# kit-cel/vae-equalizer

Measured on AMD Instinct MI355X. Metric: equalized symbols/s/GPU, DP 64-QAM VAE-LE, higher is better.
Workload: dtype f32

## Files before the change

### vae_equalizer_amd/csrc/vaeq_dp_wave_kernel.h

```cpp
#pragma once
#include <hip/hip_runtime.h>
#include <stdint.h>
#include <type_traits>

#include "vaeq.h"
#include "vaeq_common.h"
#include "vaeq_launch.h"
#include "vaeq_wave.h"

#ifdef VAEQ_PHASE_STAMPS
#define VAEQ_STAMP(i) do { if (s == a.steps - 1) tst[i] = __builtin_readcyclecounter(); } while (0)
#define VAEQ_XSTAMP(i) do { if (s == a.steps - 1) tsx[i] = __builtin_readcyclecounter(); } while (0)
#else
#define VAEQ_STAMP(i) do { } while (0)
#define VAEQ_XSTAMP(i) do { } while (0)
#endif
#define VAEQ_NSTAMP 12
#ifndef VAEQ_PIPE
#define VAEQ_PIPE 1
#endif
#define VAEQ_BT_FRAMES 16
#ifndef VAEQ_WPS
#define VAEQ_WPS 2
#endif
// ... 6 lines not shown
    return __builtin_bit_cast(float, (unsigned)r[0]) + __builtin_bit_cast(float, (unsigned)r[1]);
}

struct WaveLayout {
    int Lph, Uph;
    int X, E, U, PSv, W, H, PSh, VS, MOM, RED, XG, total;
};

__host__ __device__ inline WaveLayout wave_layout(int B, int M, int NW = 1)
{
    WaveLayout l;
    const int len = 2 * B + M - 1;
    const int lph = wave_lph(len);
    l.Lph = lph;
    l.Uph = B / 2 + 1;
    int o = 0;
    auto take = [&](int bytes) { int r = o; o += (bytes + 15) & ~15; return r; };
    l.X = take(2 * 4 * lph * 8);
    l.E = take(2 * 4 * lph * 8);
    const int ubytes = 2 * 2 * l.Uph * 8, gbytes = 2 * B * 8;
    l.U = take(ubytes > gbytes ? ubytes : gbytes);
    l.PSv = take(2 * (B + 1) * 4);
    l.W = take(2 * M * 16);
    l.H = take(2 * 2 * (M + 1) * 8);
    l.PSh = take(2 * (M + 1) * 4);
    l.VS = take(2 * M * 4);
    l.MOM = take(16 * 64 * 4);
    l.RED = take(NW > 1 ? 64 * 4 : 0);
    l.XG = take((NW - 1) * 4 * 64 * 4);
    l.total = o;
    return l;
}

template <int M, bool INIT, bool PIPE = true, bool SPLIT = true>
__device__ __forceinline__ void pair_fir(cacc (&acc)[2][2], cacc (&accx)[2][2], const float2 *xp, int Lph, const float4 *wq)
{
    cacc (&acc2)[2][2] = SPLIT ? accx : acc;
    auto tapA = [&](int k) -> v2f { return lds2(reinterpret_cast<const float2 *>(wq + k)); };
    auto tapB = [&](int k) -> v2f { return lds2(reinterpret_cast<const float2 *>(wq + k) + 1); };
    constexpr int G = M / 4;
    auto load = [&](int g, v2f (&r)[14]) {
        const float2 *xg = xp + g;
        r[0] = lds2(xg); r[1] = lds2(xg + Lph); r[2] = lds2(xg + 2 * Lph); r[3] = lds2(xg + 3 * Lph); r[4] = lds2(xg + 1); r[5] = lds2(xg + Lph + 1);
#pragma unroll
        for (int t = 0; t < 4; t++) { r[6 + 2 * t] = tapA(4 * g + t); r[7 + 2 * t] = tapB(4 * g + t); }
    };
    auto fma = [&](int, const v2f (&r)[14], auto first) {
        constexpr bool F = decltype(first)::value;
        cmacf<F>(acc[0][0], r[6], r[0]); cmacf<F>(acc[0][1], r[7], r[0]); cmacf<F>(acc[1][0], r[6], r[2]); cmacf<F>(acc[1][1], r[7], r[2]);
        cmacf<F && SPLIT>(acc2[0][0], r[8], r[1]); cmacf<F && SPLIT>(acc2[0][1], r[9], r[1]);
        cmacf<F && SPLIT>(acc2[1][0], r[8], r[3]); cmacf<F && SPLIT>(acc2[1][1], r[9], r[3]);
        cmac(acc[0][0], r[10], r[2]); cmac(acc[0][1], r[11], r[2]); cmac(acc[1][0], r[10], r[4]); cmac(acc[1][1], r[11], r[4]);
        cmac(acc2[0][0], r[12], r[3]); cmac(acc2[0][1], r[13], r[3]); cmac(acc2[1][0], r[12], r[5]); cmac(acc2[1][1], r[13], r[5]);
    };
    pipe2<14, INIT, PIPE>(G, load, fma);
#pragma unroll
    for (int k = 4 * G; k < M; k++) {
        const v2f a = tapA(k), b = tapB(k);
        const v2f xa = lds2(xp + (k & 3) * Lph + (k >> 2)), xb = lds2(xp + ((k + 2) & 3) * Lph + ((k + 2) >> 2));
        if (k & 1) { cmac(acc2[0][0], a, xa); cmac(acc2[0][1], b, xa); cmac(acc2[1][0], a, xb); cmac(acc2[1][1], b, xb); }
        else { cmac(acc[0][0], a, xa); cmac(acc[0][1], b, xa); cmac(acc[1][0], a, xb); cmac(acc[1][1], b, xb); }
    }
}

template <int M, bool MERGE = true>
__device__ __forceinline__ void pair_du(cacc (&acc)[2][2][2], const float2 *ep, int Lph, const float2 *ht, int MP)
{
    constexpr int G = M / 4;
    auto load1 = [&](int chi, int g, v2f *x) {
        const float2 *xg = ep + chi * 4 * Lph + g;
        x[0] = lds2(xg); x[1] = lds2(xg + Lph); x[2] = lds2(xg + 2 * Lph); x[3] = lds2(xg + 3 * Lph); x[4] = lds2(xg + 1); x[5] = lds2(xg + Lph + 1);
#pragma unroll
        for (int t = 0; t < 4; t++) { x[6 + 2 * t] = lds2(ht + (chi * 2 + 0) * MP + 4 * g + t); x[7 + 2 * t] = lds2(ht + (chi * 2 + 1) * MP + 4 * g + t); }
    };
    auto fma1 = [&](int chi, const v2f *x, int t, auto first) {
        constexpr bool F = decltype(first)::value;
        cmacf<F>(acc[chi][0][0], x[6 + 2 * t], x[t]); cmacf<F>(acc[chi][0][1], x[7 + 2 * t], x[t]);
        cmacf<F>(acc[chi][1][0], x[6 + 2 * t], x[t + 2]); cmacf<F>(acc[chi][1][1], x[7 + 2 * t], x[t + 2]);
    };
    if constexpr (MERGE) {
        auto load = [&](int g, v2f (&r)[28]) { load1(0, g, r); load1(1, g, r + 14); };
        auto fma = [&](int, const v2f (&r)[28], auto first) {
            fma1(0, r, 0, first); fma1(1, r + 14, 0, first);
#pragma unroll
            for (int t = 1; t < 4; t++) { fma1(0, r, t, std::false_type{}); fma1(1, r + 14, t, std::false_type{}); }
        };
        pipe2<28, true, false>(G, load, fma);
    } else {
#pragma unroll
        for (int chi = 0; chi < 2; chi++) {
            auto load = [&](int g, v2f (&r)[14]) { load1(chi, g, r); };
            auto fma = [&](int, const v2f (&r)[14], auto first) {
                fma1(chi, r, 0, first);
#pragma unroll
                for (int t = 1; t < 4; t++) fma1(chi, r, t, std::false_type{});
            };
            pipe2<14, true, false>(G, load, fma);
        }
    }
#pragma unroll
    for (int k = 4 * G; k < M; k++)
#pragma unroll
        for (int chi = 0; chi < 2; chi++) {
            const float2 *xp = ep + chi * 4 * Lph;
            const v2f a = lds2(ht + (chi * 2 + 0) * MP + k), b = lds2(ht + (chi * 2 + 1) * MP + k);
            const v2f xa = lds2(xp + (k & 3) * Lph + (k >> 2)), xb = lds2(xp + ((k + 2) & 3) * Lph + ((k + 2) >> 2));
            cmac(acc[chi][0][0], a, xa); cmac(acc[chi][0][1], b, xa); cmac(acc[chi][1][0], a, xb); cmac(acc[chi][1][1], b, xb);
        }
}

constexpr bool uniform_parts(int B, int M, int NP)
{
    const int mh = M / 2, nm = 2 * B - 2 * mh;
// ... 146 lines not shown
    }
    constexpr bool LB = NST % 2 == 0;
    v2f t[6];
    if constexpr (N & 1) {
        constexpr int m = N - 1;
        t[0] = lds2(sA + SS * m); t[1] = lds2(sB + SS * m); t[2] = lds2(tA + m); t[3] = lds2(tA + TN + m); t[4] = lds2(tB + m); t[5] = lds2(tB + TN + m);
    }
    if constexpr (LB) { head(B, A, std::false_type{}); rest(B); }
    if constexpr (N & 1) {
        const v2f (&p)[12] = LB ? B : A;
        cmac(ca[1][0], p[10], t[0]); cmac(ca[1][1], p[11], t[0]); cmac(ca[0][0], t[2], t[0]); cmac(ca[0][1], t[3], t[0]);
        cmac(cb[0][0], t[4], t[1]); cmac(cb[0][1], t[5], t[1]); cmac(cb[1][0], t[2], t[1]); cmac(cb[1][1], t[3], t[1]);
    }
#pragma unroll
    for (int x = 0; x < 2; x++)
#pragma unroll
        for (int y = 0; y < 2; y++) { ca[x][y].a += cb[x][y].a; ca[x][y].b += cb[x][y].b; }
}

template <int M, int NLEV, int BT, bool PAIR, int OUT, int NW = 1, int BL = 0>
__global__ __launch_bounds__(64 * NW, VAEQ_WPS) void dp_wave_kernel(const vaeq_dp_args a)
{
    constexpr int mh = M / 2, Mh = 2 * mh, MP = M + 1;
    constexpr float LOG2E = 1.4426950408889634f, LN2 = 0.6931471805599453f;
    extern __shared__ float4 smem4[];
    char *sm = reinterpret_cast<char *>(smem4);
    const int gl = threadIdx.x, lane = NW > 1 ? (gl & 63) : gl, wv = NW > 1 ? (gl >> 6) : 0, run = blockIdx.x;
    constexpr int NT = 64 * NW, NP = 2 * NW;
    constexpr bool UNI = BT > 0 && uniform_parts(BT, M, NP);
    constexpr bool FIXL = BT > 0 || (BL > 0 && M != 13 && M != 17 && !(M == 31 && NW == 1));
    constexpr bool PIPE = VAEQ_PIPE && FIXL;
    constexpr bool WIDE = FIXL;
    constexpr bool B100 = BT == 100 && NW == 1;
    constexpr int QAUX = B100 ? 2 : 0;
    const int B = BT ? BT : a.B;
    const int BS = BT ? BT : BL ? BL : B;
    constexpr bool ODDB = BT == 0 && BL > 0;
    const int L = 2 * B, nm = L - Mh, P2 = ODDB ? (B + 1) / 2 : B / 2;
    const float rnm = 1.0f / (float)nm;
    const WaveLayout lay = wave_layout(BS, M, NW);
    const int Lph = lay.Lph, Uph = lay.Uph;
    float2 *Xs = reinterpret_cast<float2 *>(sm + lay.X), *Es = reinterpret_cast<float2 *>(sm + lay.E);
    float2 *Us = reinterpret_cast<float2 *>(sm + lay.U), *GY = Us;
    float4 *Wt = reinterpret_cast<float4 *>(sm + lay.W);
    float2 *Ht = reinterpret_cast<float2 *>(sm + lay.H);
    float *PSv = reinterpret_cast<float *>(sm + lay.PSv);
    float *PSh = reinterpret_cast<float *>(sm + lay.PSh);
    float *VS = reinterpret_cast<float *>(sm + lay.VS);
    float *RED = reinterpret_cast<float *>(sm + lay.RED), *XG = reinterpret_cast<float *>(sm + lay.XG);

    float amp[NLEV], b2[NLEV], nlogP[NLEV];
    const float nusc = a.nu_sc[run];
#pragma unroll
    for (int i = 0; i < NLEV; i++) {
        amp[i] = a.amp[i];
        b2[i] = nusc * amp[i] * amp[i] * LOG2E;
        nlogP[i] = -logf(a.P[(size_t)run * NLEV + i]);
    }
    const float var0 = a.var[run * 2 + 0], var1 = a.var[run * 2 + 1];
    const float lrW = a.lr_W[run], lrH = a.lr_h[run];

    for (int i = gl; i < (lay.W - lay.X) / 8; i += NT) Xs[i] = make_float2(0.f, 0.f);
    for (int i = gl; i < (lay.PSh - lay.H) / 8; i += NT) Ht[i] = make_float2(0.f, 0.f);
    __syncthreads();
    const int tk = lane & 31, half = lane >> 5;
    const bool worker = tk < M, owner = worker && wv == 0;
// ... 71 lines not shown
            b2t = BTW[1][f];
        }
        const bool qf = OUT != 2 && a.q_out, yf = a.y_out, ef = OUT != 1 && a.eq_out, df = OUT != 1 && a.dec_out;
        const uint32_t No4 = (uint32_t)No * 4u;
        const size_t fr = (size_t)run * a.n_frames + f;
        const __amdgpu_buffer_rsrc_t qr = make_rsrc(qf ? a.q_out + fr * (4 * NLEV) * No : nullptr, qf ? 4u * NLEV * No4 : 0u);
        const __amdgpu_buffer_rsrc_t yr = make_rsrc(yf ? a.y_out + fr * 4 * No : nullptr, yf ? 4u * No4 : 0u);
        const __amdgpu_buffer_rsrc_t er = make_rsrc(ef ? a.eq_out + fr * 2 * No : nullptr, ef ? 2u * No4 : 0u);
        const __amdgpu_buffer_rsrc_t dr = make_rsrc(df ? a.dec_out + fr * 4 * No : nullptr, df ? (uint32_t)(4 * No) : 0u);
        const __amdgpu_buffer_rsrc_t lr_ = make_rsrc(a.loss ? a.loss + fr * a.steps : nullptr, a.loss ? (uint32_t)a.steps * 4u : 0u);
        const __amdgpu_buffer_rsrc_t vr_ = make_rsrc(a.var_est ? a.var_est + fr * 2 * a.steps : nullptr, a.var_est ? (uint32_t)a.steps * 8u : 0u);
#pragma unroll 1
        for (int s = 0; s < a.steps; s++) {
            VAEQ_STAMP(0);
            if (ldl) {
#pragma unroll
                for (int p = 0; p < 2; p++) {
                    const float4 I4 = pf[p * 2 + 0], Q4 = pf[p * 2 + 1];
                    const float xi[4] = {I4.x, I4.y, I4.z, I4.w}, xq[4] = {Q4.x, Q4.y, Q4.z, Q4.w};
#pragma unroll
                    for (int i = 0; i < 4; i++) {
                        const int c = mh + i;
                        const bool in = !ODDB || 4 * gl + i < L;
                        Xs[(p * 4 + (c & 3)) * Lph + gl + (c >> 2)] = in ? make_float2(xi[i], xq[i]) : make_float2(0.f, 0.f);
                    }
                }
            }
            sync_lds<NW>();

            VAEQ_STAMP(1);
            float2 y[2][2];
            {
                cacc ya[2][2], yb[2][2];
                pair_fir<M, true, PIPE, WIDE>(ya, yb, Xa, Lph, Wt);
                pair_fir<M, false, PIPE, WIDE>(ya, yb, Xa + 4 * Lph, Lph, Wt + M);
#pragma unroll
                for (int sy = 0; sy < 2; sy++)
#pragma unroll
                    for (int o = 0; o < 2; o++) {
                        if constexpr (WIDE) {
                            ya[sy][o].a += yb[sy][o].a;
                            ya[sy][o].b += yb[sy][o].b;
                        }
                        y[sy][o] = cfin(ya[sy][o]);
                    }
            }
            asm volatile("" : "+v"(y[0][0].x), "+v"(y[0][0].y), "+v"(y[0][1].x), "+v"(y[0][1].y), "+v"(y[1][0].x), "+v"(y[1][0].y),
                         "+v"(y[1][1].x), "+v"(y[1][1].y));
            VAEQ_STAMP(2);
            const bool kept0 = act && (n0 >= k0) && (n0 < k0 + klen), kept1 = act && (n0 + 1 >= k0) && (n0 + 1 < k0 + klen);
            const uint32_t col = (uint32_t)(s * klen + (n0 - k0));
            const uint32_t vo0 = kept0 ? col * 4u : OOB, vo1 = kept1 ? col * 4u + 4u : OOB;
            if (yf) {
                uint32_t yrow = 0u;
                auto next_row = [&]() {
                    yrow += No4;
                    asm volatile("" : "+s"(yrow));
                };
#pragma unroll
                for (int o = 0; o < 2; o++) {
                    const uint32_t r0 = yrow;
                    next_row();
                    const uint32_t r1 = yrow;
                    next_row();
                    if (pairst) {
                        bst64(v2f{y[0][o].x, y[1][o].x}, yr, vo0, r0);
                        bst64(v2f{y[0][o].y, y[1][o].y}, yr, vo0, r1);
                    } else {
// ... 101 lines not shown
                    sync_lds<NW>();
#pragma unroll
                    for (int w = 0; w < NW - 1; w++)
                        if (w < wv) { inc[0] += RED[w]; inc[1] += RED[NW + w]; }
                }
#pragma unroll
                for (int o = 0; o < 2; o++) {
                    if (act) {
                        PSv[o * (BS + 1) + n0 + 1] = inc[o] - vv[o][1];
                        PSv[o * (BS + 1) + n0 + 2] = inc[o];
                    }
                    if (gl == 0) PSv[o * (BS + 1)] = 0.f;
                }
            }
            sync_lds<NW>();
            if (owner) {
                const int lo = (Mh - tk + 1) >> 1, hi_ = (nm - 1 + Mh - tk) >> 1;
                VS[half * M + tk] = PSv[half * (BS + 1) + hi_ + 1] - PSv[half * (BS + 1) + lo];
            }
            sync_lds<NW>();

            VAEQ_STAMP(5);
            float se0 = 0.f, se1 = 0.f;
            float hq0 = 0.f, hq1 = 0.f;
            if (worker) {
                const float2 h0 = Ht[(0 * 2 + half) * MP + tk], h1 = Ht[(1 * 2 + half) * MP + tk];
                hq0 = h0.x * h0.x + h0.y * h0.y;
                hq1 = h1.x * h1.x + h1.y * h1.y;
            }
            const float vsl = worker ? VS[half * M + tk] : 0.f;
            if constexpr (B100 && M == 25) {
                constexpr int T = 100 - mh, NB = (mh + 1) / 2;
                static_assert((mh & 1) == 0 && (Mh & 3) == 0 && D3Map::exact(100, M), "D3Map: mh even (a = mh stands alone, its odd tap is the pad)");
                int l3 = lane;
                asm volatile("" : "+v"(l3));
                const int m3 = D3Map::m(l3, T), modd = m3 & 1, m3h = (3 * m3) >> 1;
                cacc D3[3][2];
                const int xo = D3Map::chi(l3) * 4 * Lph + (Mh >> 2) + m3h;
                const int o0 = xo + (modd ? 2 * Lph : 0), o2 = xo + (modd ? 1 : 2 * Lph);
                const int off[6] = {o0, o0 + Lph, o2, o2 + Lph, o0 + 1, o0 + Lph + 1};
                v2f x6[6];
#pragma unroll
                for (int k = 0; k < 6; k++) x6[k] = lds2(Xs + off[k]);
                {
                    const float2 *uE = Us + modd * Uph + m3h, *uO = Us + (modd ^ 1) * Uph + m3h + modd;
                    const float2 *hc = Ht + D3Map::chi(l3) * 2 * MP;
                    v2f am[2][4];
#pragma unroll
                    for (int v = 0; v < 2; v++) {
                        am[v][0] = lds2(hc + v * MP + Mh);
                        am[v][1] = lds2(uE + v * 2 * Uph); am[v][2] = lds2(uO + v * 2 * Uph); am[v][3] = lds2(uE + v * 2 * Uph + 1);
                    }
#pragma unroll
                    for (int v = 0; v < 2; v++) {
                        const float2 *hv = hc + v * MP, *ue = uE + v * 2 * Uph, *uo = uO + v * 2 * Uph;
                        {
                            const v2f t = am[v][0], u0 = am[v][1], u1 = am[v][2], u2 = am[v][3];
                            if (v == 0) { cmul(D3[0][0], t, u0); cmul(D3[1][0], t, u1); cmul(D3[2][0], t, u2); }
                            else { cmac(D3[0][0], t, u0); cmac(D3[1][0], t, u1); cmac(D3[2][0], t, u2); }
                        }
                        auto load = [&](int b, v2f (&r)[8]) {
                            const int sl = (mh >> 1) - b;
                            r[0] = lds2(uo + sl - 1); r[1] = lds2(ue + sl); r[2] = lds2(uo + sl); r[3] = lds2(ue + sl + 1);
#pragma unroll
                            for (int t = 0; t < 4; t++) r[4 + t] = lds2(hv + 4 * b + t);
                        };
                        auto fma = [&](int, const v2f (&r)[8], auto first) {
                            constexpr bool F = decltype(first)::value;
                            v2f t0 = r[4], t1 = r[5], t2 = r[6], t3 = r[7];
                            asm volatile("" : "+v"(t0), "+v"(t1));
#pragma unroll
                            for (int i = 0; i < 3; i++) {
                                cmac(D3[i][0], t0, r[i + 1]);
                                cmacf<F>(D3[i][1], t1, r[i + 1]);
                                if constexpr (F) asm volatile("" : "+v"(D3[i][1].a), "+v"(D3[i][1].b));
                            }
                            asm volatile("" : "+v"(t2), "+v"(t3));
#pragma unroll
                            for (int i = 0; i < 3; i++) { cmac(D3[i][0], t2, r[i]); cmac(D3[i][1], t3, r[i]); }
                        };
                        if (v == 0) pipe2<8, true, PIPE>(NB, load, fma);
                        else pipe2<8, false, PIPE>(NB, load, fma);
                    }
                }
                VAEQ_STAMP(6);
                {
                    float2 e[6];
#pragma unroll
                    for (int k = 0; k < 6; k++) {
                        const float2 x = f2(x6[k]);
                        const float2 Dv = cfin(D3[k >> 1][k & 1]);
                        e[k] = make_float2(x.x - Dv.x, x.y - Dv.y);
                        if (6 * (D3Map::nm_lanes(T) - 1) + k >= 2 * T && 6 * m3 + k >= nm) e[k] = make_float2(0.f, 0.f);
                    }
                    if (D3Map::works(l3, T)) {
#pragma unroll
                        for (int k = 0; k < 6; k++) Es[off[k]] = e[k];
                    }
                }
                sync_lds<NW>();
                {
                    const float2 *Eq = Es + (gl < nq ? gl : 0);
                    v2f eq[2][4];
#pragma unroll
                    for (int chi = 0; chi < 2; chi++)
#pragma unroll
                        for (int i = 0; i < 4; i++) eq[chi][i] = lds2(Eq + (chi * 4 + ((Mh + i) & 3)) * Lph + ((Mh + i) >> 2));
#pragma unroll
                    for (int chi = 0; chi < 2; chi++)
#pragma unroll
                        for (int i = 0; i < 4; i++) {
                            const float2 e = f2(eq[chi][i]);
                            const float e2 = __builtin_fmaf(e.x, e.x, e.y * e.y);
                            if (chi) se1 += e2; else se0 += e2;
// ... 79 lines not shown
                }
            }
            {
                const float inc = half_incl_scan_dpp(gC0 * hq0 + gC1 * hq1);
                if (owner) PSh[half * MP + tk + 1] = inc;
                if (tk == 0) PSh[half * MP] = 0.f;
            }
            sync_lds<NW>();

            VAEQ_STAMP(7);
            step += 1;
            b1t *= 0.9;
            b2t *= 0.999;
            const float rbc1 = __builtin_amdgcn_rcpf((float)(1.0 - b1t));
            const float bc2s = __builtin_amdgcn_rcpf(__builtin_amdgcn_sqrtf((float)(1.0 - b2t)));
            const float ssW = lrW * rbc1, ssH = lrH * rbc1;
            float2 hnew[2];
            hnew[0] = hnew[1] = make_float2(0.f, 0.f);
            float ghr[2] = {0, 0}, ghi[2] = {0, 0};
            float2 hacc[2];
            {
                float2 ph_h[2] = {make_float2(0.f, 0.f), make_float2(0.f, 0.f)};
                float ph_vs[2] = {0.f, 0.f};
                if (NW == 1 && ownr) {
#pragma unroll
                    for (int v = 0; v < 2; v++) {
                        ph_h[v] = Ht[(oc * 2 + v) * MP + tj];
                        ph_vs[v] = VS[v * M + tj];
                    }
                }
                cacc ca[2][2];
                if constexpr (TP) {
                    static_assert(TapPairMap::exact(100, M) && UNI, "TapPairMap");
                    int lt = lane;
                    asm volatile("" : "+v"(lt));
                    constexpr int NH = TapPairMap::dh_pairs(100, M);
                    const int par = TapPairMap::par(lt, M), sl = TapPairMap::alo(lt, M) >> 1, ma = TapPairMap::part_h(lt, M) * NH;
                    const int ceA = par + Mh, ceB = par + Mh + 2;
                    const float2 *ec = Es + TapPairMap::c(lt, M) * 4 * Lph + ma;
                    const float2 *uA = Us + (mh >> 1) - sl + ma, *uB = uA + Uph;
                    const float2 *uC = TapPairMap::tap(lt, M, 1) < M ? uB - 1 : uA;
                    VAEQ_XSTAMP(0);
                    tap_pair_sum<NH, 1>(ca, ec + (ceA & 3) * Lph + (ceA >> 2), ec + (ceB & 3) * Lph + (ceB >> 2), uA, uB, 2 * Uph, uC);
                } else {
                    const int tkc = worker ? tk : 0, par = tkc & 1, aa = tkc >> 1;
                    const int T = (nm - par + 1) >> 1, Th = ((T + 2 * NP - 1) / (2 * NP)) << 1;
                    const int ma = (part * Th) >> 1, mb = (min(T, part * Th + Th) + 1) >> 1;
                    const int ceA = par + Mh, ceB = par + Mh + 2, npA = mh - aa, npB = mh - aa + 1;
                    const float2 *eA = Es + (ceA & 3) * Lph + (ceA >> 2) + ma, *eB = Es + (ceB & 3) * Lph + (ceB >> 2) + ma;
                    const float2 *uA = Us + (npA & 1) * Uph + (npA >> 1) + ma, *uB = Us + (npB & 1) * Uph + (npB >> 1) + ma;
                    auto load1 = [&](int m, v2f *r) {
                        r[0] = lds2(eA + m); r[1] = lds2(eA + 4 * Lph + m); r[2] = lds2(uA + m); r[3] = lds2(uA + 2 * Uph + m);
                        r[4] = lds2(eB + m); r[5] = lds2(eB + 4 * Lph + m); r[6] = lds2(uB + m); r[7] = lds2(uB + 2 * Uph + m);
                    };
                    cacc cbx[2][2];
                    cacc (&cb)[2][2] = WIDE ? cbx : ca;
                    auto fma1 = [&](const v2f *r, auto first) {
                        constexpr bool F = decltype(first)::value;
                        cmacf<F>(ca[0][0], r[2], r[0]); cmacf<F>(ca[0][1], r[3], r[0]); cmacf<F>(ca[1][0], r[2], r[1]); cmacf<F>(ca[1][1], r[3], r[1]);
                        cmacf<F && WIDE>(cb[0][0], r[6], r[4]); cmacf<F && WIDE>(cb[0][1], r[7], r[4]); cmacf<F && WIDE>(cb[1][0], r[6], r[5]); cmacf<F && WIDE>(cb[1][1], r[7], r[5]);
                    };
                    auto load = [&](int i, v2f (&r)[16]) { load1(2 * i, r); load1(2 * i + 1, r + 8); };
                    auto fma = [&](int, const v2f (&r)[16], auto first) { fma1(r, first); fma1(r + 8, std::false_type{}); };
                    int n = mb - ma;
                    VAEQ_XSTAMP(0);
                    if constexpr (UNI) {
                        n = __builtin_amdgcn_readfirstlane(n);
                        pipe2<16, true, PIPE>(n >> 1, load, fma);
// ... 51 lines not shown
                    for (int v = 0; v < 2; v++) {
                        const float2 ac = half ? acc[1][v] : acc[0][v];
                        const float2 hh = ph_h[v];
                        const float vs = ph_vs[v];
                        ghr[v] = g * (-2.0f * ac.x + 2.0f * hh.x * vs);
                        ghi[v] = g * (-2.0f * ac.y + 2.0f * hh.y * vs);
                        hnew[v] = hh;
                        if (!a.no_update) {
                            adam_update_fast(hnew[v].x, mHr(v), vHr(v), ghr[v], ssH, bc2s);
                            adam_update_fast(hnew[v].y, mHi(v), vHi(v), ghi[v], ssH, bc2s);
                        }
                    }
                }
            }

            asm volatile("" : "+v"(hnew[0].x), "+v"(hnew[0].y), "+v"(hnew[1].x), "+v"(hnew[1].y), "+v"(ghr[0]), "+v"(ghr[1]), "+v"(ghi[0]),
                         "+v"(ghi[1]));
            {
                const bool last_s = s + 1 == a.steps;
                if constexpr (B100) {
                    const bool more = !(last_s && f + 1 == a.n_frames);
                    const uint32_t vo = ldl && more ? ((uint32_t)(last_s ? 0 : s + 1) * (uint32_t)a.stride_sym * 2u + 4u * gl) * 4u : OOB;
#pragma unroll
                    for (int r = 0; r < 4; r++) pf[r] = bld128(last_s ? xn : xr, vo, (uint32_t)r * S4);
                } else if (!(last_s && f + 1 == a.n_frames)) fetch(last_s ? xn : xr, last_s ? 0 : s + 1);
            }
            VAEQ_XSTAMP(3);
            VAEQ_STAMP(8);
            float2 gy[2][2];
            {
                float2 au0[2][2], au1[2][2];
                {
                    cacc cu[2][2][2];
                    pair_du<M, WIDE>(cu, Ea, Lph, Ht, MP);
#pragma unroll
                    for (int sy = 0; sy < 2; sy++)
#pragma unroll
                        for (int v = 0; v < 2; v++) { au0[sy][v] = cfinc(cu[0][sy][v]); au1[sy][v] = cfinc(cu[1][sy][v]); }
                }
#pragma unroll
                for (int sy = 0; sy < 2; sy++) {
                    const int sx = 2 * (n0 + sy);
                    const int jlo = max(0, Mh - sx), jhi = max(jlo - 1, min(Mh, nm - 1 + Mh - sx));
#pragma unroll
                    for (int v = 0; v < 2; v++) {
                        const float ur = -2.0f * (gC0 * au0[sy][v].x + gC1 * au1[sy][v].x);
                        const float ui = -2.0f * (gC0 * au0[sy][v].y + gC1 * au1[sy][v].y);
                        const float gv = PSh[v * MP + jhi + 1] - PSh[v * MP + jlo];
                        const float iv = 1.0f / (v ? var1 : var0);
                        gy[sy][v].x = iv * (ur * mv[sy][v][0] + gv * mt3[sy][v][0] + mkc[sy][v][0]);
                        gy[sy][v].y = iv * (ui * mv[sy][v][1] + gv * mt3[sy][v][1] + mkc[sy][v][1]);
                    }
                }
            }
            VAEQ_STAMP(9);
            sync_lds<NW>();
            if constexpr (NW > 1) {
                if (owner) {
                    const float g = half ? gC1 : gC0;
#pragma unroll
                    for (int v = 0; v < 2; v++) {
                        float2 ac = hacc[v];
#pragma unroll
                        for (int w = 0; w < NW - 1; w++) {
                            ac.x += XG[(w * 4 + 2 * v + 0) * 64 + lane];
                            ac.y += XG[(w * 4 + 2 * v + 1) * 64 + lane];
                        }
// ... 7 lines not shown
                            adam_update_fast(hnew[v].y, mHi(v), vHi(v), ghi[v], ssH, bc2s);
                        }
                    }
                }
            }
            if (act) {
#pragma unroll
                for (int v = 0; v < 2; v++) {
                    GY[v * BS + n0] = gy[0][v];
                    GY[v * BS + n0 + 1] = v1 ? gy[1][v] : make_float2(0.f, 0.f);
                }
            }
            if (ownr && !a.no_update) {
                Ht[(oc * 2 + 0) * MP + tj] = hnew[0];
                Ht[(oc * 2 + 1) * MP + tj] = hnew[1];
            }
            sync_lds<NW>();

            VAEQ_STAMP(10);
            float gwr[2] = {0, 0}, gwi[2] = {0, 0};
            {
                float pw_w[2][2] = {{0.f, 0.f}, {0.f, 0.f}}, pw_m[2][2] = {{0.f, 0.f}, {0.f, 0.f}}, pw_v[2][2] = {{0.f, 0.f}, {0.f, 0.f}};
                if (ownr) {
#pragma unroll
                    for (int p = 0; p < 2; p++) {
                        const float *wq = reinterpret_cast<const float *>(&Wt[p * M + tj]) + oc * 2;
                        pw_w[p][0] = wq[0]; pw_w[p][1] = wq[1];
                        pw_m[p][0] = mWr(p); pw_m[p][1] = mWi(p);
                        pw_v[p][0] = vWr(p); pw_v[p][1] = vWi(p);
                    }
                }
                cacc ca[2][2];
                if constexpr (TP) {
                    int lt = lane;
                    asm volatile("" : "+v"(lt));
                    constexpr int NQ = TapPairMap::dw_pairs(100);
                    const int cA = TapPairMap::tap(lt, M, 1), cB = cA + 2, ma = TapPairMap::part_w(lt) * NQ;
                    const float2 *gA = GY + TapPairMap::c(lt, M) * BS + 2 * ma;
                    const float2 *xA = Xs + (cA & 3) * Lph + (cA >> 2) + ma, *xB = Xs + (cB & 3) * Lph + (cB >> 2) + ma;
                    cacc cr[2][2];
                    VAEQ_XSTAMP(4);
                    tap_pair_sum<NQ, 2>(cr, gA, gA + 1, xA, xB, 4 * Lph, xB - 1);
#pragma unroll
                    for (int p = 0; p < 2; p++) { ca[0][p] = cr[1][p]; ca[1][p] = cr[0][p]; }
                } else {
                    const int tkc = worker ? tk : 0;
                    const int Be = ODDB ? B + (B & 1) : B;
                    const int Bq = ((Be + 2 * NP - 1) / (2 * NP)) << 1;
                    const int ma = (part * Bq) >> 1, mb = min(Be, part * Bq + Bq) >> 1;
                    const int cA = tkc, cB = tkc + 2;
                    const float2 *xA = Xs + (cA & 3) * Lph + (cA >> 2) + ma, *xB = Xs + (cB & 3) * Lph + (cB >> 2) + ma;
                    const float2 *G0 = GY + 2 * ma, *G1 = GY + BS + 2 * ma;
                    auto load1 = [&](int m, v2f *r) {
                        r[0] = lds2(G0 + 2 * m); r[1] = lds2(G0 + 2 * m + 1); r[2] = lds2(G1 + 2 * m); r[3] = lds2(G1 + 2 * m + 1);
                        r[4] = lds2(xA + m); r[5] = lds2(xA + 4 * Lph + m); r[6] = lds2(xB + m); r[7] = lds2(xB + 4 * Lph + m);
                    };
                    cacc cbx[2][2];
                    cacc (&cb)[2][2] = WIDE ? cbx : ca;
                    auto fma1 = [&](const v2f *r, auto first) {
                        constexpr bool F = decltype(first)::value;
                        cmacf<F>(ca[0][0], r[4], r[0]); cmacf<F>(ca[0][1], r[5], r[0]); cmacf<F>(ca[1][0], r[4], r[2]); cmacf<F>(ca[1][1], r[5], r[2]);
                        cmacf<F && WIDE>(cb[0][0], r[6], r[1]); cmacf<F && WIDE>(cb[0][1], r[7], r[1]); cmacf<F && WIDE>(cb[1][0], r[6], r[3]); cmacf<F && WIDE>(cb[1][1], r[7], r[3]);
                    };
                    auto load = [&](int i, v2f (&r)[16]) { load1(2 * i, r); load1(2 * i + 1, r + 8); };
                    auto fma = [&](int, const v2f (&r)[16], auto first) { fma1(r, first); fma1(r + 8, std::false_type{}); };
                    int n = mb - ma;
                    VAEQ_XSTAMP(4);
                    if constexpr (UNI) {
// ... 201 lines not shown
```

### vae_equalizer_amd/csrc/vaeq_wave.h

```cpp
#pragma once
#include <hip/hip_runtime.h>
#include <stdint.h>
#include <type_traits>

namespace vaeq {

__device__ __forceinline__ void wave_lds_sync() { asm volatile("" ::: "memory"); }

template <int NW>
__device__ __forceinline__ void sync_lds()
{
    if constexpr (NW == 1) wave_lds_sync();
    else asm volatile("s_waitcnt lgkmcnt(0)\n\ts_barrier" ::: "memory");
}

template <int NW, int K>
__device__ __forceinline__ void waves_sum(float (&v)[K], float *red, int lane, int wv)
{
    if constexpr (NW > 1) {
        if (lane == 0) {
#pragma unroll
            for (int k = 0; k < K; k++) red[k * NW + wv] = v[k];
        }
        sync_lds<NW>();
// ... 78 lines not shown
    return __builtin_bit_cast(float4, v);
}

template <int NR, bool INIT, bool PIPE = true, class L, class F>
__device__ __forceinline__ void pipe2(int n, L load, F fma)
{
    if (!INIT && n <= 0) return;
    if constexpr (!PIPE) {
        v2f A[NR];
        load(0, A);
        fma(0, A, std::integral_constant<bool, INIT>{});
#pragma unroll 1
        for (int i = 1; i < n; i++) {
            load(i, A);
            fma(i, A, std::false_type{});
        }
        return;
    }
    v2f A[NR], B[NR];
    load(0, A);
    load(1, B);
    fma(0, A, std::integral_constant<bool, INIT>{});
    int i = 1;
#pragma unroll 1
    for (; i + 1 < n; i += 2) {
        load(i + 1, A);
        fma(i, B, std::false_type{});
        load(i + 2, B);
        fma(i + 1, A, std::false_type{});
    }
    if (i < n) fma(i, B, std::false_type{});
}

__device__ __forceinline__ v2f cfin2(const cacc &c)
{
    v2f r;
    asm("v_pk_add_f32 %0, %1, %2 op_sel:[0,1] op_sel_hi:[1,0] neg_lo:[0,1]" : "=v"(r) : "v"(c.a), "v"(c.b));
    return r;
}
__device__ __forceinline__ v2f cfinc2(const cacc &c)
{
    v2f r;
    asm("v_pk_add_f32 %0, %1, %2 op_sel:[0,1] op_sel_hi:[1,0] neg_hi:[0,1]" : "=v"(r) : "v"(c.a), "v"(c.b));
    return r;
}
__device__ __forceinline__ float2 cfin(const cacc &c) { const v2f r = cfin2(c); return make_float2(r.x, r.y); }
__device__ __forceinline__ float2 cfinc(const cacc &c) { const v2f r = cfinc2(c); return make_float2(r.x, r.y); }

template <int CTRL, int ROW_MASK = 0xF, int BANK_MASK = 0xF>
__device__ __forceinline__ float dpp_f(float v)
{
    return __builtin_bit_cast(float, __builtin_amdgcn_update_dpp(0, __builtin_bit_cast(int, v), CTRL, ROW_MASK, BANK_MASK, true));
}
__device__ __forceinline__ float wave_sum_dpp(float v)
{
    v += dpp_f<0xB1>(v);
    v += dpp_f<0x4E>(v);
    v += dpp_f<0x141>(v);
    v += dpp_f<0x140>(v);
    v += dpp_f<0x142, 0xA>(v);
    v += dpp_f<0x143, 0xC>(v);
    return __builtin_bit_cast(float, __builtin_amdgcn_readlane(__builtin_bit_cast(int, v), 63));
}
__device__ __forceinline__ float row_incl_scan_dpp(float v)
{
    float s = v + dpp_f<0x111>(v);
// ... 38 lines not shown
```

Baseline: 10.99 billion.

## Carry overlapping LDS cells across pipelined FIR, dL/dU and D-stage iterations

Adds a carried variant of the software-pipelined loop (pipe2_carry) that reuses the x/e/mu cells already loaded for the previous tap group instead of reloading them from LDS. It is enabled for the B=100, M=25 single-wave path in the FIR, pair_du and D3 stages, with constexpr checks that the carried offsets match the original reads exactly. It also removes asm barriers that pinned lane indices. The change cuts LDS read traffic per tap group, at the cost of more live registers and a more rigid schedule that could affect occupancy.

```diff
diff --git a/vae_equalizer_amd/csrc/vaeq_dp_wave_kernel.h b/vae_equalizer_amd/csrc/vaeq_dp_wave_kernel.h
--- a/vae_equalizer_amd/csrc/vaeq_dp_wave_kernel.h
+++ b/vae_equalizer_amd/csrc/vaeq_dp_wave_kernel.h
@@ -62,9 +62,86 @@
     return l;
 }
 
-template <int M, bool INIT, bool PIPE = true, bool SPLIT = true>
+struct CellCarry {
+    static constexpr int fir_off(int g, int j, int Lph) { return g + (j < 4 ? j * Lph : (j - 4) * Lph + 1); }
+    static constexpr int poly4(int c, int Lph) { return (c & 3) * Lph + (c >> 2); }
+    static constexpr int d3_off(int b, int d, int mh, int Uph) { return (d & 1 ? Uph : 0) + (mh >> 1) - b + (d == -1 ? -1 : d == 2 ? 1 : 0); }
+    static constexpr int poly2(int c, int Uph) { return (c & 1) * Uph + (c >> 1); }
+    static constexpr bool fir_exact(int B, int M)
+    {
+        const int G = M / 4, len = 2 * B + M - 1, Lph = wave_lph(len);
+        if (M % 4 != 1 || G < 2 || G % 2) return false;
+        for (int g = 0; g < G; g++)
+            for (int j = 0; j < 6; j++) {
+                if (fir_off(g, j, Lph) != poly4(4 * g + j, Lph)) return false;
+                if (4 * (B / 2 - 1) + 4 * g + j >= len) return false;
+                if (g + 1 < G && j >= 4 && fir_off(g, j, Lph) != fir_off(g + 1, j - 4, Lph)) return false;
+            }
+        return poly4(4 * G, Lph) == fir_off(G - 1, 4, Lph) && 4 * (B / 2 - 1) + 4 * G + 2 < len;
+    }
+    static constexpr bool d3_exact(int B, int M)
+    {
+        const int mh = M / 2, NB = (mh + 1) / 2, Uph = B / 2 + 1, T = B - mh;
+        if ((mh & 1) || NB < 2 || NB % 2) return false;
+        for (int b = 0; b < NB; b++)
+            for (int d = -1; d <= 2; d++) {
+                if (d3_off(b, d, mh, Uph) != poly2(mh - 2 * b + d, Uph)) return false;
+                if (mh - 2 * b + d < 0 || 3 * (D3Map_nm_lanes(T) - 1) + mh - 2 * b + d >= 2 * Uph) return false;
+                if (b + 1 < NB && d <= 0 && d3_off(b, d, mh, Uph) != d3_off(b + 1, d + 2, mh, Uph)) return false;
+            }
+        return true;
+    }
+    static constexpr int D3Map_nm_lanes(int T) { return (T + 2) / 3; }
+};
+static_assert(CellCarry::fir_exact(100, 25), "B = 100: the FIR / dL/dU stages must carry exactly the cells the next stage would have read, inside x / e");
+static_assert(CellCarry::d3_exact(100, 25), "B = 100: the D stages must carry exactly the mu cells the next stage would have read, inside U");
+
+template <int M, bool INIT>
+__device__ __forceinline__ void pair_fir_carry(cacc (&acc)[2][2], cacc (&acc2)[2][2], const float2 *xp, int Lph, const float4 *wq)
+{
+    constexpr int G = M / 4;
+    auto tapA = [&](int k) -> v2f { return lds2(reinterpret_cast<const float2 *>(wq + k)); };
+    auto tapB = [&](int k) -> v2f { return lds2(reinterpret_cast<const float2 *>(wq + k) + 1); };
+    auto taps = [&](int g, v2f (&r)[14]) {
+#pragma unroll
+        for (int t = 0; t < 4; t++) { r[6 + 2 * t] = tapA(4 * g + t); r[7 + 2 * t] = tapB(4 * g + t); }
+    };
+    auto loadF = [&](v2f (&r)[14]) {
+        r[0] = lds2(xp); r[1] = lds2(xp + Lph); r[2] = lds2(xp + 2 * Lph); r[3] = lds2(xp + 3 * Lph); r[4] = lds2(xp + 1); r[5] = lds2(xp + Lph + 1);
+        taps(0, r);
+    };
+    auto loadM = [&](int g, v2f (&r)[14]) { r[2] = lds2(xp + g + 2 * Lph); r[3] = lds2(xp + g + 3 * Lph); taps(g, r); };
+    auto loadL = [&](int g, v2f (&r)[14]) { r[4] = lds2(xp + g + 1); r[5] = lds2(xp + g + Lph + 1); };
+    auto fma0 = [&](const v2f (&r)[14]) {
+        cmacf<INIT>(acc[0][0], r[6], r[0]); cmacf<INIT>(acc[0][1], r[7], r[0]); cmacf<INIT>(acc[1][0], r[6], r[2]); cmacf<INIT>(acc[1][1], r[7], r[2]);
+        cmacf<INIT>(acc2[0][0], r[8], r[1]); cmacf<INIT>(acc2[0][1], r[9], r[1]); cmacf<INIT>(acc2[1][0], r[8], r[3]); cmacf<INIT>(acc2[1][1], r[9], r[3]);
+        cmac(acc[0][0], r[10], r[2]); cmac(acc[0][1], r[11], r[2]); cmac(acc[1][0], r[10], r[4]); cmac(acc[1][1], r[11], r[4]);
+        cmac(acc2[0][0], r[12], r[3]); cmac(acc2[0][1], r[13], r[3]); cmac(acc2[1][0], r[12], r[5]); cmac(acc2[1][1], r[13], r[5]);
+    };
+    auto stage = [&](const v2f (&r)[14], const v2f (&p)[14], auto mid) {
+        cmac(acc[0][0], r[6], p[4]); cmac(acc[0][1], r[7], p[4]); cmac(acc2[0][0], r[8], p[5]); cmac(acc2[0][1], r[9], p[5]);
+        asm volatile("" : "+v"(acc[0][0].a), "+v"(acc[0][0].b), "+v"(acc[0][1].a), "+v"(acc[0][1].b), "+v"(acc2[0][0].a), "+v"(acc2[0][0].b),
+                     "+v"(acc2[0][1].a), "+v"(acc2[0][1].b));
+        mid();
+        cmac(acc[1][0], r[6], r[2]); cmac(acc[1][1], r[7], r[2]); cmac(acc2[1][0], r[8], r[3]); cmac(acc2[1][1], r[9], r[3]);
+        cmac(acc[0][0], r[10], r[2]); cmac(acc[0][1], r[11], r[2]); cmac(acc[1][0], r[10], r[4]); cmac(acc[1][1], r[11], r[4]);
+        cmac(acc2[0][0], r[12], r[3]); cmac(acc2[0][1], r[13], r[3]); cmac(acc2[1][0], r[12], r[5]); cmac(acc2[1][1], r[13], r[5]);
+    };
+    constexpr int k = 4 * G;
+    v2f ta, tb, xb;
+    auto pre = [&]() { ta = tapA(k); tb = tapB(k); xb = lds2(xp + ((k + 2) & 3) * Lph + ((k + 2) >> 2)); };
+    auto post = [&](const v2f (&r)[14]) { cmac(acc[0][0], ta, r[4]); cmac(acc[0][1], tb, r[4]); cmac(acc[1][0], ta, xb); cmac(acc[1][1], tb, xb); };
+    pipe2_carry<14>(G, loadF, loadM, loadL, fma0, stage, pre, post);
+}
+
+template <int M, bool INIT, bool PIPE = true, bool SPLIT = true, bool CARRY = false>
 __device__ __forceinline__ void pair_fir(cacc (&acc)[2][2], cacc (&accx)[2][2], const float2 *xp, int Lph, const float4 *wq)
 {
+    if constexpr (CARRY) {
+        static_assert(PIPE && SPLIT, "the carried form is the pipelined, split one");
+        pair_fir_carry<M, INIT>(acc, accx, xp, Lph, wq);
+        return;
+    }
     cacc (&acc2)[2][2] = SPLIT ? accx : acc;
     auto tapA = [&](int k) -> v2f { return lds2(reinterpret_cast<const float2 *>(wq + k)); };
     auto tapB = [&](int k) -> v2f { return lds2(reinterpret_cast<const float2 *>(wq + k) + 1); };
@@ -93,7 +170,7 @@
     }
 }
 
-template <int M, bool MERGE = true>
+template <int M, bool MERGE = true, bool CARRY = false>
 __device__ __forceinline__ void pair_du(cacc (&acc)[2][2][2], const float2 *ep, int Lph, const float2 *ht, int MP)
 {
     constexpr int G = M / 4;
@@ -108,7 +185,59 @@
         cmacf<F>(acc[chi][0][0], x[6 + 2 * t], x[t]); cmacf<F>(acc[chi][0][1], x[7 + 2 * t], x[t]);
         cmacf<F>(acc[chi][1][0], x[6 + 2 * t], x[t + 2]); cmacf<F>(acc[chi][1][1], x[7 + 2 * t], x[t + 2]);
     };
-    if constexpr (MERGE) {
+    if constexpr (CARRY) {
+        static_assert(MERGE && M % 4 == 1, "the carried form is the merged one, with one tap left over");
+        auto loadF = [&](v2f (&r)[28]) { load1(0, 0, r); load1(1, 0, r + 14); };
+        auto loadM = [&](int g, v2f (&r)[28]) {
+#pragma unroll
+            for (int chi = 0; chi < 2; chi++) {
+                const float2 *xg = ep + chi * 4 * Lph + g;
+                v2f *x = r + 14 * chi;
+                x[2] = lds2(xg + 2 * Lph); x[3] = lds2(xg + 3 * Lph);
+#pragma unroll
+                for (int t = 0; t < 4; t++) { x[6 + 2 * t] = lds2(ht + (chi * 2 + 0) * MP + 4 * g + t); x[7 + 2 * t] = lds2(ht + (chi * 2 + 1) * MP + 4 * g + t); }
+            }
+        };
+        auto loadL = [&](int g, v2f (&r)[28]) {
+#pragma unroll
+            for (int chi = 0; chi < 2; chi++) { r[14 * chi + 4] = lds2(ep + chi * 4 * Lph + g + 1); r[14 * chi + 5] = lds2(ep + chi * 4 * Lph + g + Lph + 1); }
+        };
+        auto fma0 = [&](const v2f (&r)[28]) {
+            fma1(0, r, 0, std::true_type{}); fma1(1, r + 14, 0, std::true_type{});
+#pragma unroll
+            for (int t = 1; t < 4; t++) { fma1(0, r, t, std::false_type{}); fma1(1, r + 14, t, std::false_type{}); }
+        };
+        auto stage = [&](const v2f (&r)[28], const v2f (&p)[28], auto) {
+#pragma unroll
+            for (int t = 0; t < 2; t++)
+#pragma unroll
+                for (int chi = 0; chi < 2; chi++) {
+                    const v2f *x = r + 14 * chi;
+                    cmac(acc[chi][0][0], x[6 + 2 * t], p[14 * chi + 4 + t]); cmac(acc[chi][0][1], x[7 + 2 * t], p[14 * chi + 4 + t]);
+                    cmac(acc[chi][1][0], x[6 + 2 * t], x[t + 2]); cmac(acc[chi][1][1], x[7 + 2 * t], x[t + 2]);
+                }
+#pragma unroll
+            for (int t = 2; t < 4; t++) { fma1(0, r, t, std::false_type{}); fma1(1, r + 14, t, std::false_type{}); }
+        };
+        constexpr int k = 4 * G;
+        v2f ta[2], tb[2], xb[2];
+        auto pre = [&]() {
+#pragma unroll
+            for (int chi = 0; chi < 2; chi++) {
+                ta[chi] = lds2(ht + (chi * 2 + 0) * MP + k); tb[chi] = lds2(ht + (chi * 2 + 1) * MP + k);
+                xb[chi] = lds2(ep + chi * 4 * Lph + ((k + 2) & 3) * Lph + ((k + 2) >> 2));
+            }
+        };
+        auto post = [&](const v2f (&r)[28]) {
+#pragma unroll
+            for (int chi = 0; chi < 2; chi++) {
+                cmac(acc[chi][0][0], ta[chi], r[14 * chi + 4]); cmac(acc[chi][0][1], tb[chi], r[14 * chi + 4]);
+                cmac(acc[chi][1][0], ta[chi], xb[chi]); cmac(acc[chi][1][1], tb[chi], xb[chi]);
+            }
+        };
+        pipe2_carry<28, false>(G, loadF, loadM, loadL, fma0, stage, pre, post);
+        return;
+    } else if constexpr (MERGE) {
         auto load = [&](int g, v2f (&r)[28]) { load1(0, g, r); load1(1, g, r + 14); };
         auto fma = [&](int, const v2f (&r)[28], auto first) {
             fma1(0, r, 0, first); fma1(1, r + 14, 0, first);
@@ -321,6 +450,7 @@
     constexpr bool PIPE = VAEQ_PIPE && FIXL;
     constexpr bool WIDE = FIXL;
     constexpr bool B100 = BT == 100 && NW == 1;
+    constexpr bool CARRY = B100 && M == 25 && PIPE && WIDE;
     constexpr int QAUX = B100 ? 2 : 0;
     const int B = BT ? BT : a.B;
     const int BS = BT ? BT : BL ? BL : B;
@@ -458,8 +588,8 @@
             float2 y[2][2];
             {
                 cacc ya[2][2], yb[2][2];
-                pair_fir<M, true, PIPE, WIDE>(ya, yb, Xa, Lph, Wt);
-                pair_fir<M, false, PIPE, WIDE>(ya, yb, Xa + 4 * Lph, Lph, Wt + M);
+                pair_fir<M, true, PIPE, WIDE, CARRY>(ya, yb, Xa, Lph, Wt);
+                pair_fir<M, false, PIPE, WIDE, CARRY>(ya, yb, Xa + 4 * Lph, Lph, Wt + M);
 #pragma unroll
                 for (int sy = 0; sy < 2; sy++)
 #pragma unroll
@@ -627,8 +757,7 @@
             if constexpr (B100 && M == 25) {
                 constexpr int T = 100 - mh, NB = (mh + 1) / 2;
                 static_assert((mh & 1) == 0 && (Mh & 3) == 0 && D3Map::exact(100, M), "D3Map: mh even (a = mh stands alone, its odd tap is the pad)");
-                int l3 = lane;
-                asm volatile("" : "+v"(l3));
+                const int l3 = lane;
                 const int m3 = D3Map::m(l3, T), modd = m3 & 1, m3h = (3 * m3) >> 1;
                 cacc D3[3][2];
                 const int xo = D3Map::chi(l3) * 4 * Lph + (Mh >> 2) + m3h;
@@ -674,7 +803,30 @@
 #pragma unroll
                             for (int i = 0; i < 3; i++) { cmac(D3[i][0], t2, r[i]); cmac(D3[i][1], t3, r[i]); }
                         };
-                        if (v == 0) pipe2<8, true, PIPE>(NB, load, fma);
+                        if constexpr (CARRY) {
+                            static_assert(CellCarry::d3_exact(100, M) && CellCarry::D3Map_nm_lanes(T) == D3Map::nm_lanes(T), "CellCarry");
+                            auto loadF = [&](v2f (&r)[8]) { load(0, r); };
+                            auto loadM = [&](int b, v2f (&r)[8]) {
+#pragma unroll
+                                for (int t = 0; t < 4; t++) r[4 + t] = lds2(hv + 4 * b + t);
+                            };
+                            auto loadL = [&](int b, v2f (&r)[8]) { const int sl = (mh >> 1) - b; r[0] = lds2(uo + sl - 1); r[1] = lds2(ue + sl); };
+                            auto stage = [&](const v2f (&r)[8], const v2f (&p)[8], auto mid) {
+                                v2f t0 = r[4], t1 = r[5], t2 = r[6], t3 = r[7];
+                                asm volatile("" : "+v"(t0), "+v"(t1), "+v"(t2), "+v"(t3));
+                                cmac(D3[2][0], t0, p[1]); cmac(D3[2][1], t1, p[1]); cmac(D3[1][0], t0, p[0]); cmac(D3[1][1], t1, p[0]);
+                                cmac(D3[2][0], t2, p[0]); cmac(D3[2][1], t3, p[0]);
+                                asm volatile("" : "+v"(D3[1][0].a), "+v"(D3[1][0].b), "+v"(D3[1][1].a), "+v"(D3[1][1].b), "+v"(D3[2][0].a), "+v"(D3[2][0].b),
+                                             "+v"(D3[2][1].a), "+v"(D3[2][1].b));
+                                mid();
+                                cmac(D3[0][0], t0, r[1]); cmac(D3[0][1], t1, r[1]); cmac(D3[1][0], t2, r[1]); cmac(D3[1][1], t3, r[1]);
+                                cmac(D3[0][0], t2, r[0]); cmac(D3[0][1], t3, r[0]);
+                            };
+                            auto none = [&]() {};
+                            auto done = [&](const v2f (&)[8]) {};
+                            if (v == 0) pipe2_carry<8>(NB, loadF, loadM, loadL, [&](const v2f (&r)[8]) { fma(0, r, std::true_type{}); }, stage, none, done);
+                            else pipe2_carry<8>(NB, loadF, loadM, loadL, [&](const v2f (&r)[8]) { fma(0, r, std::false_type{}); }, stage, none, done);
+                        } else if (v == 0) pipe2<8, true, PIPE>(NB, load, fma);
                         else pipe2<8, false, PIPE>(NB, load, fma);
                     }
                 }
@@ -820,8 +972,7 @@
                 cacc ca[2][2];
                 if constexpr (TP) {
                     static_assert(TapPairMap::exact(100, M) && UNI, "TapPairMap");
-                    int lt = lane;
-                    asm volatile("" : "+v"(lt));
+                    const int lt = lane;
                     constexpr int NH = TapPairMap::dh_pairs(100, M);
                     const int par = TapPairMap::par(lt, M), sl = TapPairMap::alo(lt, M) >> 1, ma = TapPairMap::part_h(lt, M) * NH;
                     const int ceA = par + Mh, ceB = par + Mh + 2;
@@ -939,7 +1090,7 @@
                 float2 au0[2][2], au1[2][2];
                 {
                     cacc cu[2][2][2];
-                    pair_du<M, WIDE>(cu, Ea, Lph, Ht, MP);
+                    pair_du<M, WIDE, CARRY>(cu, Ea, Lph, Ht, MP);
 #pragma unroll
                     for (int sy = 0; sy < 2; sy++)
 #pragma unroll
@@ -1013,8 +1164,7 @@
                 }
                 cacc ca[2][2];
                 if constexpr (TP) {
-                    int lt = lane;
-                    asm volatile("" : "+v"(lt));
+                    const int lt = lane;
                     constexpr int NQ = TapPairMap::dw_pairs(100);
                     const int cA = TapPairMap::tap(lt, M, 1), cB = cA + 2, ma = TapPairMap::part_w(lt) * NQ;
                     const float2 *gA = GY + TapPairMap::c(lt, M) * BS + 2 * ma;
diff --git a/vae_equalizer_amd/csrc/vaeq_wave.h b/vae_equalizer_amd/csrc/vaeq_wave.h
--- a/vae_equalizer_amd/csrc/vaeq_wave.h
+++ b/vae_equalizer_amd/csrc/vaeq_wave.h
@@ -134,6 +134,46 @@
     if (i < n) fma(i, B, std::false_type{});
 }
 
+template <int NR, bool PIPE = true, class LF, class LM, class LL, class F0, class S, class PRE, class POST>
+__device__ __forceinline__ void pipe2_carry(int n, LF loadF, LM loadM, LL loadL, F0 fma0, S stage, PRE pre, POST post)
+{
+    v2f A[NR], B[NR];
+    loadF(A);
+    if constexpr (!PIPE) {
+        fma0(A);
+        int i = 1;
+#pragma unroll 1
+        for (; i + 1 < n; i += 2) {
+            loadM(i, B);
+            loadL(i, B);
+            stage(B, A, []() {});
+            loadM(i + 1, A);
+            loadL(i + 1, A);
+            stage(A, B, []() {});
+        }
+        loadM(i, B);
+        loadL(i, B);
+        stage(B, A, []() {});
+        pre();
+        post(B);
+        return;
+    }
+    loadM(1, B);
+    loadL(1, B);
+    fma0(A);
+    int i = 1;
+#pragma unroll 1
+    for (; i + 1 < n; i += 2) {
+        loadM(i + 1, A);
+        stage(B, A, [&]() { loadL(i + 1, A); });
+        loadM(i + 2, B);
+        stage(A, B, [&]() { loadL(i + 2, B); });
+    }
+    pre();
+    stage(B, A, []() {});
+    post(B);
+}
+
 __device__ __forceinline__ v2f cfin2(const cacc &c)
 {
     v2f r;
```

Result: faster. 11.35 billion (median of 6 runs) (+3.3%).
